# catniplab/vlgp

Hardware: AMD Instinct MI355X
Metric: EM iterations/sec (higher is better)
Workload: dtype f64

## Files before the change

### vlgp_amd/csrc/api.hip

```cpp
#include <stdarg.h>
#include <stdio.h>
#include <stdlib.h>
#include <string.h>

#include <chrono>

#include <algorithm>
#include <new>

#include "ctx.h"

static thread_local std::string g_create_err;

int vlgp_fail(vlgp_ctx* ctx, int code, const char* fmt, ...) {
    char buf[1024];
    va_list ap;
    va_start(ap, fmt);
    vsnprintf(buf, sizeof(buf), fmt, ap);
    va_end(ap);
    if (ctx) ctx->err = buf;
    else g_create_err = buf;
    return code;
}

// ... 117 lines not shown
    if (us->is(a.kinds)) return VLGP_OK;
    if (us->is(SET_REPLICATED) && &a != &admit_vlgp_replicate)
        return vlgp_fail(ctx, VLGP_ERR_STATE, "%s refuses a replicated set (leave-one-out replicas of set %d: "
                         "E-step, download, loglik and free only)", a.what, us->rep.src);
    return vlgp_fail(ctx, VLGP_ERR_STATE, a.refusal, set);
}

enum : unsigned {
    OPEN_COLLECT = 1,
    OPEN_STALE = 2,
    OPEN_JOIN = 4,
    OPEN_WAIT = 8,
    OPEN_PARAMS = 16,
    OPEN_DEVICE = 32,
    OPEN_EMPTY = 64,
};
#define NEED_PARAMS(ctx) \
    if (!(ctx)->have_params) return vlgp_fail(ctx, VLGP_ERR_STATE, "parameters not set (vlgp_set_params)")
static int open_set(vlgp_ctx* ctx, int set, unsigned how, UnitSet** out, const Admission* a) {
    NEED_CTX(ctx);
    if (how & OPEN_COLLECT) CHK(vlgp_prior_collect(ctx));
    if (how & OPEN_STALE) ctx->hmom_us = nullptr;
    if (how & OPEN_JOIN) CHK(vlgp_join_m(ctx));
    if (how & OPEN_WAIT) {
        CHK(wait_norms(ctx));
        if (ctx->m_pending) HIPCHK(ctx, hipEventSynchronize(ctx->ev_m_done));
    }
    if (how & OPEN_PARAMS) NEED_PARAMS(ctx);
    if (how & OPEN_DEVICE) HIPCHK(ctx, hipSetDevice(ctx->dev));
    if (!(*out = vlgp_get_set(ctx, set, !(how & OPEN_EMPTY)))) return VLGP_ERR_ARG;
    return a ? admit(ctx, set, *out, *a) : VLGP_OK;
}
static int open_pair(vlgp_ctx* ctx, int src, int dst, bool bad_args, const char* bad, UnitSet** s, UnitSet** d) {
    CHK(open_set(ctx, src, OPEN_STALE | OPEN_JOIN | OPEN_DEVICE, s, nullptr));
    if (!(*d = vlgp_get_set(ctx, dst, false))) return VLGP_ERR_ARG;
// ... 51 lines not shown

static void free_set(vlgp_ctx* ctx, UnitSet& us) {
    if (!us.valid) return;
    (void)hipStreamSynchronize(ctx->stream);
    auto fr = [](void* p) { if (p) (void)hipFree(p); };
    if (us.is(SET_REPLICATED)) {
        Replicas& r = us.rep;
        fr(us.mu); fr(us.v); fr(us.w); fr(r.d_ch); fr(r.d_pair); fr(r.d_mask); fr(r.d_wconst); fr(r.d_nobs); fr(r.d_xa);
        ctx->sets[r.src].rep_users--;
        us.d_xb = nullptr;
    } else if (!us.alias) {
        fr(us.y); fr(us.x); fr(us.mu); fr(us.v); fr(us.w);
    }
    fr(us.dmu); fr(us.d_off); fr(us.d_src_start); fr(us.d_unit_prior); fr(us.d_xb); fr(us.d_scratch); fr(us.d_mu_stash);
    fr(us.d_links);
    us = UnitSet();
}

static void free_with_tiling_cuts(vlgp_ctx* ctx, int set) {
    for (auto& other : ctx->sets)
        if (other.valid && other.is(SET_TILING) && other.parent == set) free_set(ctx, other);
    free_set(ctx, ctx->sets[set]);
}

extern "C" int vlgp_create(int device, int N, int L, int P, int R, const uint8_t* gauss_mask, vlgp_ctx** out) {
    if (!out) return vlgp_fail(nullptr, VLGP_ERR_ARG, "null output handle");
    *out = nullptr;
    if (N < 1 || L < 1 || P < 1 || R < 1) return vlgp_fail(nullptr, VLGP_ERR_ARG, "N, L, P, R must be positive");
    if (R > VLGP_MAX_RANK) return vlgp_fail(nullptr, VLGP_ERR_ARG, "rank %d exceeds VLGP_MAX_RANK=%d", R, VLGP_MAX_RANK);
    if (L > VLGP_MAX_L) return vlgp_fail(nullptr, VLGP_ERR_ARG, "at most %d latents supported, got %d", VLGP_MAX_L, L);
// ... 740 lines not shown
            return vlgp_fail(ctx, VLGP_ERR_STATE, "no prior factor for unit length %d (call build_prior/set_prior)", T);
        idx[m] = it->second.index;
    }
    HIPCHK(ctx, hipMemcpy(us.d_unit_prior, idx.data(), sizeof(int) * us.M, hipMemcpyHostToDevice));
    us.prior_epoch = ctx->prior_epoch;
    return VLGP_OK;
}

int vlgp_refresh_xb(vlgp_ctx* ctx, UnitSet& us) {
    if (us.x_ones) return VLGP_OK;
    if (!us.d_xb) HIPCHK(ctx, hipMalloc(&us.d_xb, (size_t)us.rows * ctx->N * sizeof(double)));
    return launch_xb(ctx, us);
}

static int begin_count(vlgp_ctx* ctx) {
    HIPCHK(ctx, hipMemsetAsync(ctx->d_fail, 0, sizeof(int), ctx->stream));
    return VLGP_OK;
}
static int end_count(vlgp_ctx* ctx, int* n_failed) {
    if (!n_failed) return VLGP_OK;
    HIPCHK(ctx, hipMemcpyAsync(n_failed, ctx->d_fail, sizeof(int), hipMemcpyDeviceToHost, ctx->stream));
    HIPCHK(ctx, hipStreamSynchronize(ctx->stream));
    return VLGP_OK;
}

extern "C" int vlgp_update_w(vlgp_ctx* ctx, int set) {
    UnitSet* us = nullptr;
    CHK(open_set(ctx, set, OPEN_COLLECT | OPEN_STALE | OPEN_JOIN | OPEN_PARAMS | OPEN_DEVICE, &us, &admit_vlgp_update_w));
    return launch_estep(ctx, *us, EM_W, 0, 0.0, 0);
}

extern "C" int vlgp_update_v(vlgp_ctx* ctx, int set, int vb, int* n_failed) {
    UnitSet* us = nullptr;
    CHK(open_set(ctx, set, OPEN_COLLECT | OPEN_JOIN | OPEN_PARAMS | OPEN_DEVICE, &us, &admit_vlgp_update_v));
    if (n_failed) *n_failed = 0;
    if (!vb) return VLGP_OK;
    CHK(begin_count(ctx));
    CHK(launch_estep(ctx, *us, EM_FACTOR0 | EM_V, 0, 0.0, 1));
    return end_count(ctx, n_failed);
}

static int estep_staged(vlgp_ctx* ctx, UnitSet& us, int mode, int n_iter, double dmu_bound, int vb) {
    const int W = us.Tmax, N = ctx->N, L = ctx->L, P = ctx->P;
    CHK(vlgp_bind_priors(ctx, us));
    const int n_stages = (int)us.stage_start.size() - 1;
    for (int s = 0; s < n_stages; ++s) {
        const int u0 = us.stage_start[s], cnt = us.stage_start[s + 1] - u0;
        if (cnt < 1) continue;
        CHK(launch_links_copy(ctx, us, us.link_start[s], us.link_start[s + 1], 0));
        UnitSet v;
        v.valid = true; v.M = cnt; v.rows = (int64_t)cnt * W; v.Tmax = v.Tmin = W;
        v.off.resize(cnt + 1);
        for (int m = 0; m <= cnt; ++m) v.off[m] = (int64_t)m * W;
        v.d_off = us.d_off;
        const int64_t r0 = (int64_t)u0 * W;
        v.y = us.y + r0 * N; v.x = us.x ? us.x + r0 * P * N : nullptr;
        v.mu = us.mu + r0 * L; v.v = us.v + r0 * L; v.w = us.w + r0 * L; v.dmu = us.dmu + r0 * L;
        v.x_ones = us.x_ones; v.alias = true;
// ... 1 lines not shown
        if (!us.x_ones) {
            if (!us.d_xb) HIPCHK(ctx, hipMalloc(&us.d_xb, (size_t)us.rows * N * sizeof(double)));
            v.d_xb = us.d_xb + r0 * N;
        }
        v.d_scratch = us.d_scratch; v.scratch_len = us.scratch_len;
        const int rc = launch_estep(ctx, v, mode, n_iter, dmu_bound, vb);
        us.d_scratch = v.d_scratch; us.scratch_len = v.scratch_len;
        if (rc != VLGP_OK) return rc;
        CHK(launch_links_copy(ctx, us, us.link_start[s], us.link_start[s + 1], 1));
    }
    return VLGP_OK;
}

extern "C" int vlgp_estep(vlgp_ctx* ctx, int set, int n_iter, double dmu_bound, int vb, int* n_failed) {
    UnitSet* us = nullptr;
    CHK(open_set(ctx, set, OPEN_COLLECT | OPEN_STALE | OPEN_JOIN | OPEN_PARAMS | OPEN_DEVICE, &us, &admit_vlgp_estep));
    if (n_failed) *n_failed = 0;
    if (n_iter < 1) return VLGP_OK;
    if (!(dmu_bound > 0)) return vlgp_fail(ctx, VLGP_ERR_ARG, "dmu_bound must be positive");
    CHK(begin_count(ctx));
    const int mode = EM_FACTOR0 | EM_MEAN | EM_W | (vb ? EM_V : 0);
    if (us->stage_start.size() > 2) CHK(estep_staged(ctx, *us, mode, n_iter, dmu_bound, vb ? 1 : 0));
    else CHK(launch_estep(ctx, *us, mode, n_iter, dmu_bound, vb ? 1 : 0));
    if (!ctx->ev_e_done) HIPCHK(ctx, hipEventCreateWithFlags(&ctx->ev_e_done, hipEventDisableTiming));
    HIPCHK(ctx, hipEventRecord(ctx->ev_e_done, ctx->stream));
    ctx->e_done_valid = true;
    return end_count(ctx, n_failed);
}

extern "C" int vlgp_set_overlaps(vlgp_ctx* ctx, int set, int n_stages, const int* stage_start, int n_links,
                                 const int* links, const int* link_start) {
// ... 142 lines not shown
        ctx->last_h_ms = std::chrono::duration<double, std::milli>(std::chrono::steady_clock::now().time_since_epoch()).count() - ctx->h_t0;
    ctx->hmom_bracket = false;
    ctx->hmom_us = nullptr;
    ctx->hwlm_valid = false;
    return VLGP_OK;
}

extern "C" int vlgp_apply_latent_map(vlgp_ctx* ctx, int set, const double* map, const double* shift) {
    NEED_CTX(ctx);
    ctx->hmom_us = nullptr;
    CHK(vlgp_join_m(ctx));
    HIPCHK(ctx, hipSetDevice(ctx->dev));
    UnitSet* us = vlgp_get_set(ctx, set, true);
    if (!us || !map) return vlgp_fail(ctx, VLGP_ERR_ARG, "bad latent map arguments");
    CHK(admit(ctx, set, us, admit_vlgp_apply_latent_map));
    const int L = ctx->L;
    if (!ctx->h_stage_map) {
        HIPCHK(ctx, hipHostMalloc(&ctx->h_stage_map, sizeof(double) * (L * L + L + 8), hipHostMallocDefault));
        HIPCHK(ctx, hipMalloc(&ctx->d_stage_map, sizeof(double) * (L * L + L + 8)));
        HIPCHK(ctx, hipEventCreateWithFlags(&ctx->ev_stage_map, hipEventDisableTiming));
    }
    if (ctx->stage_map_busy) HIPCHK(ctx, hipEventSynchronize(ctx->ev_stage_map));
    memcpy(ctx->h_stage_map, map, sizeof(double) * L * L);
    if (shift) memcpy(ctx->h_stage_map + L * L, shift, sizeof(double) * L);
    HIPCHK(ctx, hipMemcpyAsync(ctx->d_stage_map, ctx->h_stage_map, sizeof(double) * (L * L + L), hipMemcpyHostToDevice, ctx->stream));
    const double* d_map = ctx->d_stage_map;
    const double* d_shift = shift ? ctx->d_stage_map + L * L : nullptr;
    CHK(launch_latent_map(ctx, *us, d_map, d_shift));
    CHK(launch_links_map(ctx, *us, d_map, d_shift));
    HIPCHK(ctx, hipEventRecord(ctx->ev_stage_map, ctx->stream));
    ctx->stage_map_busy = true;
    return VLGP_OK;
}

static int moments_host(vlgp_ctx* ctx, UnitSet& us, std::vector<double>& out) {
    const int L = ctx->L;
    const int K = L * (L + 1) / 2 + 3 * L + 1;
    CHK(vlgp_ensure_pinned(ctx, K + 8));
    CHK(launch_moments(ctx, us));
    HIPCHK(ctx, hipMemcpyAsync(ctx->h_pinned, ctx->d_work, sizeof(double) * K, hipMemcpyDeviceToHost, ctx->stream));
    HIPCHK(ctx, hipStreamSynchronize(ctx->stream));
    out.assign(ctx->h_pinned, ctx->h_pinned + K);
// ... 274 lines not shown
```

### vlgp_amd/csrc/ctx.h

```cpp
#pragma once
#include <hip/hip_runtime.h>
#include <stdint.h>

#include <map>
#include <string>
#include <vector>

#include "../../include/vlgp_hip.h"

#define VLGP_WAVE 64
#define VLGP_E_LANES 4
#define VLGP_PRIOR_SLOTS 64

struct Prior {
    int T = 0;
    double* d_full = nullptr;
    double* d_compact = nullptr;
    std::vector<int> rl;
    std::vector<int64_t> goff;
    int64_t compact_len = 0;
    int index = -1;
};

enum : unsigned {
// ... 157 lines not shown
    double* d_hres = nullptr;
    unsigned h_seq = 0;
    double* d_hmpart = nullptr;
    bool hprep = false;
    hipEvent_t ev_e_done = nullptr;
    bool e_done_valid = false;
    uint64_t hprep_epoch = 0, write_epoch = 0;
    double* d_hmom = nullptr;
    int64_t hmom_len = 0;
    const UnitSet* hmom_us = nullptr;
    int hmom_T = 0;
    bool hmom_bracket = false;
    double* d_hwlm = nullptr;
    int64_t hwlm_len = 0;
    bool hwlm_valid = false;
    struct LrThr { int T; double dt, tol; std::vector<double> om; };
    std::vector<LrThr> lr_thr;
    Switches sw;
    std::vector<const void*> lds_attr_done;
    int h_prio = 1;
    double last_h_ms = 0.0, last_m_ms = 0.0;
    double h_t0 = 0.0;
    int last_hstep_path = 0;
    double hstat[4] = {0.0, 0.0, 0.0, 0.0};

    bool prof_on = false;
    ProfSlot prof[VLGP_PROF_KINDS];
    hipEvent_t ev0 = nullptr, ev1 = nullptr;
    struct PendingProf { int kind; hipEvent_t a, b; double units; bool done; };
    std::vector<PendingProf> pending;
// ... 9 lines not shown

    double* d_xwork = nullptr;
    double* h_xres = nullptr;
    double* d_xres = nullptr;
    unsigned long long x_seq = 0;
    int x_pending = 0;
    int x_set = -1;
    double* h_msnap = nullptr;
    double* d_msnap = nullptr;
    bool msnap_valid = false;
    double* h_stage_par = nullptr;
    double* h_stage_map = nullptr;
    double* d_stage_map = nullptr;
    hipEvent_t ev_stage_par = nullptr, ev_stage_map = nullptr;
    bool stage_par_busy = false, stage_map_busy = false;

    double* d_elbo = nullptr;
    int64_t elbo_len = 0;

    std::string err;
};

inline UnitSet& vlgp_rows_owner(vlgp_ctx* ctx, UnitSet& us) { return us.rep.src >= 0 ? ctx->sets[us.rep.src] : us; }

struct LoglikShape { int64_t slots, n_rate; int grid_y; const char* limit; };
inline LoglikShape vlgp_loglik_shape(const vlgp_ctx* ctx, const UnitSet& us) {
    if (us.is(SET_BY_ROW))
        return {(int64_t)us.rep.n * ctx->N, us.rep.rows_src * ctx->N, us.rep.n, "vlgp_loglik: at most 65535 replicas per masked set"};
    if (us.is(SET_GROUPS))
        return {us.rep.n_pairs, us.rep.rows_src * us.rep.n_pairs, us.rep.n_pairs,
// ... 48 lines not shown
static_assert(EP_LEN == VLGP_ESTEP_PLAN_LEN, "vlgp_debug_estep_plan: the report's length is part of the ABI");
int launch_mstep(vlgp_ctx* ctx, UnitSet& us, int n_iter, int use_hessian, double eps, double lr,
                 double da_bound, double db_bound);
int mstep_plan_report(vlgp_ctx* ctx, int64_t rows, int out[12]);
int launch_hstep(vlgp_ctx* ctx, UnitSet& us, int window, double dt, int n_eval, const int* latent,
                 const double* logp, double* ll, double* dll);
int launch_ichol_all(vlgp_ctx* ctx, const std::vector<Prior*>& prs, const double* omega, const double* sigma,
                     bool in_table, bool lazy = false);
int vlgp_prior_collect(vlgp_ctx* ctx);
int launch_compact_prior(vlgp_ctx* ctx, Prior& pr);
int launch_sample_posterior(vlgp_ctx* ctx, int T, int n, const double* d_mu, const double* d_w, const double* d_G,
                            const double* d_eps, double* d_z, double* d_out);
int launch_npx_probe(vlgp_ctx* ctx, int kind, int64_t n, const double* d_a, const double* d_b, double* d_out);
int launch_xb(vlgp_ctx* ctx, UnitSet& us);
int launch_latent_map(vlgp_ctx* ctx, UnitSet& us, const double* d_map, const double* d_shift);
int launch_snapshot_params(vlgp_ctx* ctx, hipStream_t st, double* d_host);
int launch_norms(vlgp_ctx* ctx, UnitSet& us, double* d_part, unsigned* d_ticket, double* d_host, unsigned long long seq);
int launch_links_copy(vlgp_ctx* ctx, UnitSet& us, int l0, int l1, int dir);
int launch_links_map(vlgp_ctx* ctx, UnitSet& us, const double* d_map, const double* d_shift);
int hstep_prepare(vlgp_ctx* ctx, UnitSet& us, int T, hipStream_t st);
int launch_moments(vlgp_ctx* ctx, UnitSet& us);
int launch_project(vlgp_ctx* ctx, UnitSet& us, const double* d_proj, const double* d_shift, double* d_part,
                   double* d_out);
int launch_gather(vlgp_ctx* ctx, UnitSet& src, UnitSet& dst, int window);
int launch_loglik(vlgp_ctx* ctx, UnitSet& us, int vb, double* d_rate, double* d_sums);
int launch_sums_finish(vlgp_ctx* ctx, int slots, int n_blk, const double* d_part, double* d_sums);
int launch_scatter(vlgp_ctx* ctx, UnitSet& cut, UnitSet& dst, int window);
int launch_elbo(vlgp_ctx* ctx, UnitSet& us, int vb, int rp, double* d_part, double* d_sums, double* d_row_ell,
                double* d_terms, int* d_flag);
int launch_forecast(vlgp_ctx* ctx, UnitSet& us, int vb, int rp, double* d_z, const int64_t* d_ext_off,
// ... 3 lines not shown
```

### vlgp_amd/csrc/estep.hip

```cpp
#include "ctx.h"

#include "estep_args.h"
#include "fast_exp.h"

__device__ __forceinline__ void wave_sync() {
    __builtin_amdgcn_fence(__ATOMIC_ACQ_REL, "workgroup");
    __builtin_amdgcn_wave_barrier();
}

__device__ __forceinline__ double shfl_xor_f64(double x, int m) { return __shfl_xor(x, m, 64); }

enum { PASS_YA = 0, PASS_RES = 1, PASS_W = 2 };

template <bool SMALL, int LT>
__global__ void __launch_bounds__(SMALL ? 512 : 1024) estep_kernel(EstepArgs A) {
    extern __shared__ __attribute__((aligned(16))) double smem[];
    const int tid = threadIdx.x, nthr = blockDim.x;
    const int lane = tid & 63, wid = tid >> 6, nw = nthr >> 6;
    const int N = A.N, L = A.L;
    const int m = blockIdx.x;
    const int64_t r0 = A.off[m];
    const int T = (int)(A.off[m + 1] - r0);
    const int pidx = A.unit_prior ? A.unit_prior[m] : -1;
    const double* Gbase = pidx >= 0 ? A.prior_base[pidx] : nullptr;
// ... 370 lines not shown

struct SmallPlan { bool fits; int nthr; int64_t d; };
static SmallPlan plan_generic_small(const UnitSet& us, int L, int64_t common, int64_t gsz, int64_t lcsz, int64_t ints,
                                    int64_t lds_max) {
    const int nw_s = L < 4 ? 4 : (L > 8 ? 8 : L);
    const int64_t small_d = common + 2LL * nw_s * 64 + 6LL * us.Tmax * L + gsz + lcsz + ints;
    return SmallPlan{us.Tmax <= 256 && small_d * 8 <= lds_max, nw_s * 64, small_d};
}

int launch_estep(vlgp_ctx* ctx, UnitSet& us, int mode, int n_iter, double dmu_bound, int vb, int* report) {
    const int N = ctx->N, L = ctx->L;
    const bool need_prior = (mode & (EM_FACTOR0 | EM_MEAN | EM_V)) != 0;
    if (need_prior) CHK(vlgp_bind_priors(ctx, us));
    if (report) {
    } else {
        UnitSet& src = vlgp_rows_owner(ctx, us);
        if (!src.x_ones) CHK(vlgp_refresh_xb(ctx, src));
        us.d_xb = src.d_xb;
    }

    const RankSummary rs = need_prior ? estep_rank_summary(ctx, us) : RankSummary();
    const int64_t gsz = rs.g_odd, lcsz = rs.lc_odd;

    const int64_t LDS_MAX = 160 * 1024;
    const int LTl = generic_lt(L);
    const int64_t common = 2LL * LTl * N + 2LL * N + ((L + 1) & ~1);
    const int64_t ints = ((int64_t)N + 4 * L + 1) / 2 + 1;

    EstepArgs A;
    A.N = N; A.L = L;
// ... 5 lines not shown
    A.a = ctx->d_a; A.b = ctx->d_b; A.noise = ctx->d_noise; A.gauss = ctx->d_gauss;
    A.scratch = nullptr; A.lc_global = nullptr; A.lc_stride = 0;
    A.fail = ctx->d_fail;
    A.clk = ctx->d_clk;
    A.cols_g = nullptr; A.wconst_g = nullptr;
    A.lds_T = us.Tmax; A.lds_gsz = (int)gsz; A.lds_lcsz = (int)lcsz;

    int* path = report ? &report[EP_FAMILY] : &ctx->last_estep_path;

    {
        int handled = 0;
        CHK(launch_estep_split(ctx, us, A, rs, &handled, report));
        if (handled) { *path = handled == 2 ? VLGP_PATH_ESTEP_LSPLIT : (handled == 3 ? VLGP_PATH_ESTEP_SPLIT_MIXED : VLGP_PATH_ESTEP_SPLIT); return VLGP_OK; }
        if (us.is(SET_REPLICATED))
            return vlgp_fail(ctx, VLGP_ERR_STATE, "replicated set: only the split E-step leaves a channel out, and it declined");
    }

    {
        int handled = 0;
        CHK(launch_estep_fast(ctx, us, A, rs, &handled, report));
        if (handled) { *path = VLGP_PATH_ESTEP_FAST; return VLGP_OK; }
    }

    if (us.Tmax > 64) {
        int handled = 0;
        CHK(launch_estep_long(ctx, us, A, &handled, report));
        if (handled) { *path = VLGP_PATH_ESTEP_LONG; return VLGP_OK; }
    }

    const SmallPlan sp = plan_generic_small(us, L, common, gsz, lcsz, ints, LDS_MAX);
// ... 51 lines not shown
```

### vlgp_amd/csrc/estep_split.hip

```cpp
#include <stdlib.h>
#include <string.h>

#include <algorithm>

#include <type_traits>

#include "estep_args.h"
#include "wave_tri.h"
#include "fast_exp.h"

namespace {

enum { SP_YA = 0, SP_RES = 1, SP_W = 2 };
typedef double double4_t __attribute__((ext_vector_type(4)));

struct ExclArgs;
struct SplitArgs {
    int N, L, M;
    int64_t rows;
    const int64_t* off;
    const int* unit_prior;
    const double* const* prior_base;
    const int* prior_rl;
    const int64_t* prior_goff;
// ... 32 lines not shown
struct ExclArgs {
    const unsigned long long* mask;
    const double* wconst;
    const double* y;
    const double* xb;
    int64_t rows_src;
    int64_t row_base;
    const double* mu_lm;
};
__host__ __device__ inline int excl_words(int N) { return (N + 63) >> 6; }
enum { EX_BY_ROW = 64 };

template <int LT>
constexpr int rec_len() { return (2 * LT + 3 + 1) & ~1; }

__global__ void __launch_bounds__(256)
esplit_cols_kernel(int N, int L, int LT, int REC, const double* __restrict__ a, const double* __restrict__ b,
                   const double* __restrict__ noise, const int* __restrict__ gauss, double* __restrict__ cols,
                   double* __restrict__ wconst, double* __restrict__ ycoef) {
    __shared__ int order[1024];
    __shared__ int gs[1024];
    __shared__ double cinv[1024];
    for (int n = threadIdx.x; n < N; n += 256) {
        const int g = gauss[n];
        gs[n] = g;
        cinv[n] = g ? 1.0 / noise[n] : 1.0;
    }
    __syncthreads();
    {
        int total = 0;
        for (int m = 0; m < N; ++m) total += gs[m];
        for (int n = threadIdx.x; n < N; n += 256) {
            int c = 0;
            for (int m = 0; m < n; ++m) c += gs[m];
// ... 55 lines not shown
__global__ void __launch_bounds__(256)
esplit_row_wconst(int N, int L, int64_t rows, int nw, const double* __restrict__ a, const double* __restrict__ noise,
                  const int* __restrict__ gauss, const unsigned long long* __restrict__ mask,
                  double* __restrict__ wconst) {
    const int64_t row = (int64_t)blockIdx.x * 256 + threadIdx.x;
    if (row >= rows) return;
    const unsigned long long* mk = mask + row * nw;
    for (int l = 0; l < L; ++l) {
        double s = 0.0;
        for (int n = 0; n < N; ++n)
            if (gauss[n] && !((mk[n >> 6] >> (n & 63)) & 1ull)) s = fma(a[l * N + n] * a[l * N + n], 1.0 / noise[n], s);
        wconst[row * L + l] = s;
    }
}

__global__ void __launch_bounds__(256)
esplit_to_lm(int L, int64_t rows, const double* __restrict__ a0, const double* __restrict__ a1,
             const double* __restrict__ a2, double* __restrict__ b0, double* __restrict__ b1, double* __restrict__ b2) {
    const int64_t row = (int64_t)blockIdx.x * 256 + threadIdx.x;
    if (row >= rows) return;
    for (int l = 0; l < L; ++l) {
        const double x0 = a0[row * L + l], x1 = a1[row * L + l], x2 = a2[row * L + l];
        b0[l * rows + row] = x0;
        b1[l * rows + row] = x1;
        b2[l * rows + row] = x2;
    }
}
__global__ void __launch_bounds__(256)
esplit_from_lm(int L, int64_t rows, const double* __restrict__ b0, const double* __restrict__ b1,
               const double* __restrict__ b2, double* a0, double* a1, double* a2) {
    const int64_t i = (int64_t)blockIdx.x * 256 + threadIdx.x;
    if (i >= rows * L) return;
    const int64_t row = i / L, l = i - row * L;
    const int64_t src = l * rows + row;
    a0[i] = b0[src];
    a1[i] = b1[src];
    a2[i] = b2[src];
}
// ... 1701 lines not shown
    const int N = ctx->N, L = ctx->L, LT = P.LT, pkg = P.pkg, n_lanes = P.n_lanes, n_it = P.n_it;
    const bool lng = P.lng;
    const LatentClasses& C = P.C;
    const int64_t nRL = P.nRL;
    if (us.scratch_len < P.scratch_len) {
        if (us.d_scratch) HIPCHK(ctx, hipFree(us.d_scratch));
        us.d_scratch = nullptr;
        us.scratch_len = 0;
        HIPCHK(ctx, hipMalloc(&us.d_scratch, (size_t)P.scratch_len * 8));
        us.scratch_len = P.scratch_len;
    }
    if (!ctx->d_ecols) HIPCHK(ctx, hipMalloc(&ctx->d_ecols, sizeof(double) * ((size_t)N * 50 + 32)));
    double* cols = ctx->d_ecols;
    double* wconst = ctx->d_ecols + (int64_t)N * 34;
    double* ycoef = wconst + 32;
    hipLaunchKernelGGL(esplit_cols_kernel, dim3(1), dim3(256), 0, ctx->stream, N, L, LT, P.REC, ctx->d_a, ctx->d_b,
                       ctx->d_noise, ctx->d_gauss, cols, wconst, ycoef);
    HIPCHK(ctx, hipGetLastError());
    ExclArgs XA{};
    if (rep) {
        XA.mask = us.rep.d_mask;
        XA.wconst = us.rep.d_wconst;
        XA.y = vlgp_rows_owner(ctx, us).y;
        XA.xb = E.xb;
        XA.rows_src = us.rep.rows_src;
        XA.row_base = 0;
        XA.mu_lm = nullptr;
        if (!by_row)
            hipLaunchKernelGGL(esplit_excl_wconst, dim3((unsigned)((us.rep.n * 16 + 255) / 256)), dim3(256), 0, ctx->stream, N,
                               L, us.rep.n, us.rep.nw, ctx->d_a, ctx->d_noise, ctx->d_gauss, us.rep.d_mask, us.rep.d_wconst);
        else if (us.rep.d_wconst)
            hipLaunchKernelGGL(esplit_row_wconst, dim3((unsigned)((us.rows + 255) / 256)), dim3(256), 0, ctx->stream, N, L,
                               us.rows, us.rep.nw, ctx->d_a, ctx->d_noise, ctx->d_gauss, us.rep.d_mask, us.rep.d_wconst);
        HIPCHK(ctx, hipGetLastError());
    }

    SplitArgs A;
    A.N = N; A.L = L; A.M = us.M; A.rows = us.rows;
    A.off = E.off; A.unit_prior = E.unit_prior; A.prior_base = E.prior_base; A.prior_rl = E.prior_rl;
    A.prior_goff = E.prior_goff;
    A.y = E.y; A.xb = E.xb; A.dmu = E.dmu;
    A.ld = us.rows;
    A.ra = us.d_scratch; A.ya = A.ra + nRL; A.mu = A.ya + nRL; A.v = A.mu + nRL; A.w = A.v + nRL;
    A.xg = A.w + nRL; A.pkg = pkg;
    {
        const unsigned nb = (unsigned)((us.rows + 255) / 256);
        hipLaunchKernelGGL(esplit_to_lm, dim3(nb), dim3(256), 0, ctx->stream, L, us.rows, E.mu, E.v, E.w, A.mu, A.v, A.w);
        HIPCHK(ctx, hipGetLastError());
    }
    if (rep) {
        XA.mu_lm = A.mu;
        static_assert(sizeof(ExclArgs) <= sizeof(us.rep.xh), "Replicas::xh too small for ExclArgs");
        memcpy(us.rep.xh, &XA, sizeof(ExclArgs));
        HIPCHK(ctx, hipMemcpyAsync(us.rep.d_xa, us.rep.xh, sizeof(ExclArgs), hipMemcpyHostToDevice, ctx->stream));
    }
    A.failg = reinterpret_cast<int*>(us.d_scratch + P.o_failg);
    A.xl = us.d_scratch + P.o_xl;
    A.sv = P.use_lane ? A.xl + P.xl_len : nullptr;
    A.dl = P.use_lane ? A.sv + nRL : nullptr;
    A.dmask = 0;
    A.fail = E.fail;
    A.wconst = wconst;
    A.dmu_bound = E.dmu_bound;
    A.ntot = N; A.np = N - ctx->n_gauss;
    A.lds_g = 256; A.pkl = pkg; A.n_lat = 0;
    A.shg = 0; A.shg_cap = 0; A.shg_T = 0;
    A.do_v = 0; A.last = 0;
    *handled = split_handled(P);
    HIPCHK(ctx, hipMemsetAsync(A.failg, 0, sizeof(int) * (size_t)us.M * L, ctx->stream));

    const int mode = E.mode;
    const bool with_mean = (mode & EM_MEAN) != 0;
    const int kind = lng ? VLGP_PROF_ESTEP_LONG
                         : (P.maxra <= 16 ? VLGP_PROF_ESTEP_RA16 : (P.maxra <= 24 ? VLGP_PROF_ESTEP_RA24 : VLGP_PROF_ESTEP_RA32));
    vlgp_prof_begin(ctx, kind);
    Lane main_lane{ctx->stream, rep ? &XA : nullptr, rep ? reinterpret_cast<const ExclArgs*>(us.rep.d_xa) : nullptr, by_row};
    int rc = VLGP_OK;
    if (with_mean) rc = run_ya(ctx, main_lane, A, LT, cols, ycoef);

    for (int h = 1; h < n_lanes; ++h) {
        if (ctx->elane[h - 1]) continue;
        HIPCHK(ctx, hipStreamCreateWithFlags(&ctx->elane[h - 1], hipStreamNonBlocking));
        HIPCHK(ctx, hipEventCreateWithFlags(&ctx->ev_e_join[h - 1], hipEventDisableTiming));
    }
// ... 64 lines not shown
                hf.lat.do_v = do_v ? 1 : 0;
                if (sample) vlgp_prof_begin(ctx, VLGP_PROF_ESTEP_FACTOR, ln.st);
                rc = lng ? run_latent_long(ctx, ln, hf.lat, false) : run_latent(ctx, ln, hf.lat, C, false);
                if (sample) vlgp_prof_end(ctx, VLGP_PROF_ESTEP_FACTOR, tasks, ln.st);
            }
        }
    }
    for (int h = 1; h < n_lanes; ++h) {
        (void)hipEventRecord(ctx->ev_e_join[h - 1], ctx->elane[h - 1]);
        (void)hipStreamWaitEvent(ctx->stream, ctx->ev_e_join[h - 1], 0);
    }
    if (rc == VLGP_OK) {
        const unsigned nb = (unsigned)((nRL + 255) / 256);
        hipLaunchKernelGGL(esplit_from_lm, dim3(nb), dim3(256), 0, ctx->stream, L, us.rows, A.mu, A.v, A.w, E.mu, E.v, E.w);
        if (hipGetLastError() != hipSuccess) rc = vlgp_fail(ctx, VLGP_ERR_HIP, "esplit_from_lm launch failed");
    }
    vlgp_prof_end(ctx, kind, (double)us.M * (E.n_iter > 0 ? E.n_iter : 1));
    return rc;
}
```

### vlgp_amd/csrc/hstep.hip

```cpp
#include <stdio.h>
#include <stdlib.h>
#include <string.h>

#include <algorithm>

#include "ctx.h"
#include "wave_tri.h"
#include "hstep_mfma.h"
#include "hstep_lr.h"

#define HS_MAXT 1024

struct HPrepArgs {
    int T;
    double dt;
    const double* logp;
    double* kinv;
    double* q;
    double* dk;
    double* scal;
    double* tm;
    double* km;
};

// ... 500 lines not shown
    const int64_t* off;
    const double* mu;
    const double* w;
    const double* wlm;
    int64_t wld;
    int latent[16];
    double logp[48];
    double* kinv;
    double* kcol;
    double* scal;
    double* out;
};

template <int T>
__global__ void __launch_bounds__(256) hstep_moment_kernel(int L, int M, int Tr, const int64_t* off, const double* mu,
                                                           int nchunk, double* part) {
    constexpr int CW = (T * T + 255) / 256;
    constexpr int NG = (T + CW - 1) / CW;
    static_assert(T * NG <= 256, "one thread per (row, run)");
    constexpr int SG = 16;
    __shared__ __attribute__((aligned(16))) double s[SG][64];
    const int l = blockIdx.y, c = blockIdx.x, tid = threadIdx.x;
    const int per = (M + nchunk - 1) / nchunk;
    const int m0 = c * per, m1 = (m0 + per < M) ? m0 + per : M;
    const bool act = tid < T * NG;
    const int j = act ? tid % T : 0, k0 = act ? (tid / T) * CW : 0;
    double acc[CW];
#pragma unroll
    for (int i = 0; i < CW; ++i) acc[i] = 0.0;
    const int w4 = tid >> 6, t = tid & 63;
    double nx[SG / 4];
    auto fetch = [&](int m) {
#pragma unroll
        for (int q = 0; q < SG / 4; ++q) {
            const int sg = w4 + 4 * q;
            nx[q] = (m + sg < m1 && t < Tr) ? mu[(off[m + sg] + t) * L + l] : 0.0;
        }
    };
    if (m0 < m1) fetch(m0);
    for (int m = m0; m < m1; m += SG) {
        __syncthreads();
#pragma unroll
        for (int q = 0; q < SG / 4; ++q) s[w4 + 4 * q][t] = nx[q];
        __syncthreads();
        if (m + SG < m1) fetch(m + SG);
#pragma unroll
        for (int sg = 0; sg < SG; ++sg) {
            const double a = s[sg][j];
#pragma unroll
            for (int i = 0; i < CW; ++i) acc[i] = fma(a, (k0 + i < 64) ? s[sg][k0 + i] : 0.0, acc[i]);
        }
// ... 389 lines not shown
    return VLGP_OK;
}

static int launch_hstep_impl(vlgp_ctx* ctx, UnitSet& us, int window, double dt, int n_eval, const int* latent,
                             const double* logp, double* ll, double* dll, bool force_dense);

int launch_hstep(vlgp_ctx* ctx, UnitSet& us, int window, double dt, int n_eval, const int* latent,
                 const double* logp, double* ll, double* dll) {
    return launch_hstep_impl(ctx, us, window, dt, n_eval, latent, logp, ll, dll, false);
}

static bool hstep_round_kernels_apply(vlgp_ctx* ctx, const UnitSet& us, int T) {
    const Switches& sw = ctx->sw;
    return us.Tmin == T && us.Tmax == T && T <= 64 && T >= (sw.hstep_dense ? 24 : 4) && !sw.hstep_generic;
}
static int hstep_prepare_units(vlgp_ctx* ctx, UnitSet& us, int T, bool want_wlm, bool want_mom, hipStream_t st) {
    const int L = ctx->L, M = us.M;
    if (want_wlm && (!ctx->hwlm_valid || ctx->hmom_us != &us)) {
        const int64_t n = us.rows * L;
        if (ctx->hwlm_len < n) {
            if (ctx->d_hwlm) HIPCHK(ctx, hipFree(ctx->d_hwlm));
            ctx->d_hwlm = nullptr; ctx->hwlm_len = 0;
            HIPCHK(ctx, hipMalloc(&ctx->d_hwlm, sizeof(double) * (size_t)n));
            ctx->hwlm_len = n;
        }
        hipLaunchKernelGGL(hstep_w_latent_major, dim3((unsigned)((n + 255) / 256)), dim3(256), 0, st, L,
                           us.rows, us.w, ctx->d_hwlm);
        HIPCHK(ctx, hipGetLastError());
        ctx->hwlm_valid = true;
    }
    if (!want_mom) return VLGP_OK;
    const int HT = T <= 50 ? 50 : 64;
    constexpr int NCH = 64;
    if (!ctx->d_hmom || ctx->hmom_len < (int64_t)L * HT * HT) {
        if (ctx->d_hmom) HIPCHK(ctx, hipFree(ctx->d_hmom));
        if (ctx->d_hmpart) HIPCHK(ctx, hipFree(ctx->d_hmpart));
        ctx->d_hmom = nullptr; ctx->d_hmpart = nullptr;
        HIPCHK(ctx, hipMalloc(&ctx->d_hmom, sizeof(double) * L * HT * HT));
        HIPCHK(ctx, hipMalloc(&ctx->d_hmpart, sizeof(double) * (size_t)L * NCH * HT * HT));
        ctx->hmom_len = (int64_t)L * HT * HT;
        ctx->hmom_us = nullptr;
    }
    if (ctx->hmom_us != &us || ctx->hmom_T != T) {
        if (HT == 50)
            hipLaunchKernelGGL((hstep_moment_kernel<50>), dim3(NCH, L), dim3(256), 0, st, L, M, T,
                               us.d_off, us.mu, NCH, ctx->d_hmpart);
        else
            hipLaunchKernelGGL((hstep_moment_kernel<64>), dim3(NCH, L), dim3(256), 0, st, L, M, T,
                               us.d_off, us.mu, NCH, ctx->d_hmpart);
        hipLaunchKernelGGL(hstep_moment_reduce, dim3((HT * HT + 255) / 256, L), dim3(256), 0, st, NCH,
                           HT * HT, ctx->d_hmpart, ctx->d_hmom);
        HIPCHK(ctx, hipGetLastError());
        ctx->hmom_us = &us;
        ctx->hmom_T = T;
    }
    return VLGP_OK;
}
int hstep_prepare(vlgp_ctx* ctx, UnitSet& us, int T, hipStream_t st) {
    if (!hstep_round_kernels_apply(ctx, us, T)) return VLGP_OK;
    ctx->hmom_us = nullptr;
    ctx->hwlm_valid = false;
    return hstep_prepare_units(ctx, us, T, !ctx->sw.hstep_no_wlm, true, st);
}

static int launch_hstep_impl(vlgp_ctx* ctx, UnitSet& us, int window, double dt, int n_eval, const int* latent,
                             const double* logp, double* ll, double* dll, bool force_dense) {
    const int T = window, L = ctx->L, M = us.M;
    if (T > HS_MAXT) return vlgp_fail(ctx, VLGP_ERR_ARG, "H-step kernel supports window <= %d, got %d", HS_MAXT, T);
    const bool huge = (size_t)(T * (T | 1)) * 8 > 150 * 1024;
    if (us.Tmin != T || us.Tmax != T)
        return vlgp_fail(ctx, VLGP_ERR_STATE, "H-step needs every unit to have exactly window=%d rows", T);
    const Switches& sw = ctx->sw;
    const bool lr_allowed = !force_dense && !sw.hstep_dense;
    const bool fast = T <= 64 && T >= (lr_allowed ? 4 : 24) && !sw.hstep_generic;
    const int TC = T <= 50 ? 50 : 64;
    const int64_t TT = fast ? (int64_t)TC * TC : (int64_t)T * T;
    const int64_t o_kinv = 0, o_q = o_kinv + n_eval * TT, o_dk = o_q + n_eval * TT, o_scal = o_dk + n_eval * TT;
// ... 11 lines not shown
    double* W = ctx->d_work;
    double* hp = ctx->h_pinned;
    if (n_eval > 16) return vlgp_fail(ctx, VLGP_ERR_ARG, "at most 16 evaluations per call, got %d", n_eval);
    for (int i = 0; i < n_eval; ++i)
        if (latent[i] < 0 || latent[i] >= L) return vlgp_fail(ctx, VLGP_ERR_ARG, "latent index out of range");

    if (fast) {
        HFastArgs F;
        F.L = L; F.M = M; F.Tr = T; F.dt = dt; F.off = us.d_off; F.mu = us.mu; F.w = us.w;
        for (int i = 0; i < n_eval; ++i) F.latent[i] = latent[i];
        for (int i = 0; i < 3 * n_eval; ++i) F.logp[i] = logp[i];
        F.kinv = W + o_kinv; F.kcol = W + o_q; F.scal = W + o_scal; F.out = W + o_out;
        F.wlm = nullptr; F.wld = 0;
        if (ctx->hmom_bracket && !sw.hstep_no_wlm) {
            CHK(hstep_prepare_units(ctx, us, T, true, false, ctx->stream));
            F.wlm = ctx->d_hwlm; F.wld = us.rows;
        }
        double* hres = hp + 4 * n_eval + 8;
        {
            if (!ctx->d_hsync) {
                HIPCHK(ctx, hipMalloc(&ctx->d_hsync, 32 * sizeof(unsigned)));
                HIPCHK(ctx, hipMemsetAsync(ctx->d_hsync, 0, 32 * sizeof(unsigned), ctx->stream));
                HIPCHK(ctx, hipHostMalloc(&ctx->h_hres, 64 * sizeof(double), hipHostMallocMapped));
                memset(ctx->h_hres, 0, 64 * sizeof(double));
                HIPCHK(ctx, hipHostGetDevicePointer(reinterpret_cast<void**>(&ctx->d_hres), ctx->h_hres, 0));
            }
            if (!ctx->hmom_bracket) ctx->hmom_us = nullptr;
            CHK(hstep_prepare_units(ctx, us, T, false, true, ctx->stream));
            HRoundArgs R;
            R.F = F;
            constexpr int MFMA_NW = 4;
// ... 274 lines not shown
```

### vlgp_amd/engine.py

```python
import collections
import ctypes as C
import logging
import os
import time

import numpy as np

from . import _lib
from ._lib import VlgpError, check, dptr, i64ptr, iptr, u8ptr

logger = logging.getLogger(__name__)

__all__ = ["Engine", "DeviceTrials", "estep", "mstep", "hstep", "update_w", "update_v",
           "make_cholesky", "infer", "vem", "constrain_loading", "constrain_latent", "VlgpError"]


TRACE = {}


def _f64(a):
    return np.ascontiguousarray(a, dtype=np.float64)


def _all_ones(x):
# ... 842 lines not shown
    def begin_m():
        if params.get("da") is None:
            params["da"] = np.zeros_like(params["a"])
            params["db"] = np.zeros_like(params["b"])
        eng.mstep_begin(sid, config["Mniter"], config["use_hessian"], config["eps"], config["learning_rate"],
                        config["da_bound"], config["db_bound"])

    early_m = m_async and not latent_constraint and not track_elbo
    if early_m:
        begin_m()
    m_first = m_async and ((eng.world > 1 and not eng.host_exchange) or bool(os.environ.get("VLGP_M_SEQUENTIAL")))

    prepare = bool(config["Hstep"]) and bool(config.get("window")) and not m_first

    def after_estep():
        eng.norms_begin(sid)
        if prepare:
            eng.hstep_prepare(sid, config["window"])

    if not latent_constraint:
        after_estep()
    eng.estep_wait()
    t1 = time.perf_counter()
    elbo_now = _elbo_totals(eng, sid, config["method"] == "VB") if track_elbo else None
    constrain_latent(trials, params, config)
    if latent_constraint:
        after_estep()
    norms_epoch = eng.state_epoch
    if m_async and not early_m:
        begin_m()

    def finish_m():
        bad, ms = eng.mstep_end()
# ... 55 lines not shown
```

Before: 154.6.

## Defer latent map and fuse it with fail-clear into split E-step prologue

The latent-map application is deferred and folded into a new fused prologue kernel that combines the column setup, the transpose to latent-major layout and the clearing of the failure counters. This removes several small launches and memsets per EM iteration. The H-step preparation now reuses the latent-major mu and w copies left behind by the split E-step instead of re-transposing them, and hstep_prepare is reordered before norms_begin. The deferral bookkeeping adds state that must be flushed correctly on every other entry path.

```diff
diff --git a/vlgp_amd/csrc/api.hip b/vlgp_amd/csrc/api.hip
--- a/vlgp_amd/csrc/api.hip
+++ b/vlgp_amd/csrc/api.hip
@@ -155,11 +155,28 @@
     OPEN_PARAMS = 16,
     OPEN_DEVICE = 32,
     OPEN_EMPTY = 64,
+    OPEN_KEEP_MAP = 128,
 };
+
+int vlgp_flush_latent_map(vlgp_ctx* ctx) {
+    if (ctx->map_pending < 0) return VLGP_OK;
+    UnitSet& us = ctx->sets[ctx->map_pending];
+    HIPCHK(ctx, hipSetDevice(ctx->dev));
+    const int L = ctx->L;
+    CHK(launch_latent_map(ctx, us, ctx->d_stage_map, ctx->map_shift ? ctx->d_stage_map + L * L : nullptr));
+    return vlgp_latent_map_consumed(ctx);
+}
+int vlgp_latent_map_consumed(vlgp_ctx* ctx) {
+    ctx->map_pending = -1;
+    HIPCHK(ctx, hipEventRecord(ctx->ev_stage_map, ctx->stream));
+    ctx->stage_map_busy = true;
+    return VLGP_OK;
+}
 #define NEED_PARAMS(ctx) \
     if (!(ctx)->have_params) return vlgp_fail(ctx, VLGP_ERR_STATE, "parameters not set (vlgp_set_params)")
 static int open_set(vlgp_ctx* ctx, int set, unsigned how, UnitSet** out, const Admission* a) {
     NEED_CTX(ctx);
+    if (!(how & OPEN_KEEP_MAP)) CHK(vlgp_flush_latent_map(ctx));
     if (how & OPEN_COLLECT) CHK(vlgp_prior_collect(ctx));
     if (how & OPEN_STALE) ctx->hmom_us = nullptr;
     if (how & OPEN_JOIN) CHK(vlgp_join_m(ctx));
@@ -241,6 +258,8 @@
     }
     fr(us.dmu); fr(us.d_off); fr(us.d_src_start); fr(us.d_unit_prior); fr(us.d_xb); fr(us.d_scratch); fr(us.d_mu_stash);
     fr(us.d_links);
+    if (ctx->lm.us == &us) ctx->lm.us = nullptr;
+    if (ctx->hwlm != ctx->d_hwlm) ctx->hwlm_valid = false;
     us = UnitSet();
 }
 
@@ -1011,10 +1030,14 @@
 }
 
 static int begin_count(vlgp_ctx* ctx) {
-    HIPCHK(ctx, hipMemsetAsync(ctx->d_fail, 0, sizeof(int), ctx->stream));
+    ctx->fail_clear = true;
     return VLGP_OK;
 }
 static int end_count(vlgp_ctx* ctx, int* n_failed) {
+    if (ctx->fail_clear) {
+        ctx->fail_clear = false;
+        HIPCHK(ctx, hipMemsetAsync(ctx->d_fail, 0, sizeof(int), ctx->stream));
+    }
     if (!n_failed) return VLGP_OK;
     HIPCHK(ctx, hipMemcpyAsync(n_failed, ctx->d_fail, sizeof(int), hipMemcpyDeviceToHost, ctx->stream));
     HIPCHK(ctx, hipStreamSynchronize(ctx->stream));
@@ -1023,13 +1046,13 @@
 
 extern "C" int vlgp_update_w(vlgp_ctx* ctx, int set) {
     UnitSet* us = nullptr;
-    CHK(open_set(ctx, set, OPEN_COLLECT | OPEN_STALE | OPEN_JOIN | OPEN_PARAMS | OPEN_DEVICE, &us, &admit_vlgp_update_w));
+    CHK(open_set(ctx, set, OPEN_COLLECT | OPEN_STALE | OPEN_JOIN | OPEN_PARAMS | OPEN_DEVICE | OPEN_KEEP_MAP, &us, &admit_vlgp_update_w));
     return launch_estep(ctx, *us, EM_W, 0, 0.0, 0);
 }
 
 extern "C" int vlgp_update_v(vlgp_ctx* ctx, int set, int vb, int* n_failed) {
     UnitSet* us = nullptr;
-    CHK(open_set(ctx, set, OPEN_COLLECT | OPEN_JOIN | OPEN_PARAMS | OPEN_DEVICE, &us, &admit_vlgp_update_v));
+    CHK(open_set(ctx, set, OPEN_COLLECT | OPEN_JOIN | OPEN_PARAMS | OPEN_DEVICE | OPEN_KEEP_MAP, &us, &admit_vlgp_update_v));
     if (n_failed) *n_failed = 0;
     if (!vb) return VLGP_OK;
     CHK(begin_count(ctx));
@@ -1039,6 +1062,7 @@
 
 static int estep_staged(vlgp_ctx* ctx, UnitSet& us, int mode, int n_iter, double dmu_bound, int vb) {
     const int W = us.Tmax, N = ctx->N, L = ctx->L, P = ctx->P;
+    CHK(vlgp_flush_latent_map(ctx));
     CHK(vlgp_bind_priors(ctx, us));
     const int n_stages = (int)us.stage_start.size() - 1;
     for (int s = 0; s < n_stages; ++s) {
@@ -1070,7 +1094,7 @@
 
 extern "C" int vlgp_estep(vlgp_ctx* ctx, int set, int n_iter, double dmu_bound, int vb, int* n_failed) {
     UnitSet* us = nullptr;
-    CHK(open_set(ctx, set, OPEN_COLLECT | OPEN_STALE | OPEN_JOIN | OPEN_PARAMS | OPEN_DEVICE, &us, &admit_vlgp_estep));
+    CHK(open_set(ctx, set, OPEN_COLLECT | OPEN_STALE | OPEN_JOIN | OPEN_PARAMS | OPEN_DEVICE | OPEN_KEEP_MAP, &us, &admit_vlgp_estep));
     if (n_failed) *n_failed = 0;
     if (n_iter < 1) return VLGP_OK;
     if (!(dmu_bound > 0)) return vlgp_fail(ctx, VLGP_ERR_ARG, "dmu_bound must be positive");
@@ -1243,6 +1267,7 @@
     UnitSet* us = vlgp_get_set(ctx, set, true);
     if (!us || !map) return vlgp_fail(ctx, VLGP_ERR_ARG, "bad latent map arguments");
     CHK(admit(ctx, set, us, admit_vlgp_apply_latent_map));
+    CHK(vlgp_flush_latent_map(ctx));
     const int L = ctx->L;
     if (!ctx->h_stage_map) {
         HIPCHK(ctx, hipHostMalloc(&ctx->h_stage_map, sizeof(double) * (L * L + L + 8), hipHostMallocDefault));
@@ -1255,6 +1280,11 @@
     HIPCHK(ctx, hipMemcpyAsync(ctx->d_stage_map, ctx->h_stage_map, sizeof(double) * (L * L + L), hipMemcpyHostToDevice, ctx->stream));
     const double* d_map = ctx->d_stage_map;
     const double* d_shift = shift ? ctx->d_stage_map + L * L : nullptr;
+    if (us->n_links == 0 && us->stage_start.size() <= 2) {
+        ctx->map_pending = set;
+        ctx->map_shift = shift != nullptr;
+        return VLGP_OK;
+    }
     CHK(launch_latent_map(ctx, *us, d_map, d_shift));
     CHK(launch_links_map(ctx, *us, d_map, d_shift));
     HIPCHK(ctx, hipEventRecord(ctx->ev_stage_map, ctx->stream));
diff --git a/vlgp_amd/csrc/ctx.h b/vlgp_amd/csrc/ctx.h
--- a/vlgp_amd/csrc/ctx.h
+++ b/vlgp_amd/csrc/ctx.h
@@ -195,6 +195,10 @@
     double* d_hwlm = nullptr;
     int64_t hwlm_len = 0;
     bool hwlm_valid = false;
+    const double* hwlm = nullptr;
+    struct LmCopy { const UnitSet* us; uint64_t epoch; const double *mu, *w; int64_t ld; };
+    LmCopy lm = {nullptr, 0, nullptr, nullptr, 0};
+    bool fail_clear = false;
     struct LrThr { int T; double dt, tol; std::vector<double> om; };
     std::vector<LrThr> lr_thr;
     Switches sw;
@@ -234,6 +238,8 @@
     double* d_stage_map = nullptr;
     hipEvent_t ev_stage_par = nullptr, ev_stage_map = nullptr;
     bool stage_par_busy = false, stage_map_busy = false;
+    int map_pending = -1;
+    bool map_shift = false;
 
     double* d_elbo = nullptr;
     int64_t elbo_len = 0;
@@ -312,6 +318,8 @@
 int launch_npx_probe(vlgp_ctx* ctx, int kind, int64_t n, const double* d_a, const double* d_b, double* d_out);
 int launch_xb(vlgp_ctx* ctx, UnitSet& us);
 int launch_latent_map(vlgp_ctx* ctx, UnitSet& us, const double* d_map, const double* d_shift);
+int vlgp_flush_latent_map(vlgp_ctx* ctx);
+int vlgp_latent_map_consumed(vlgp_ctx* ctx);
 int launch_snapshot_params(vlgp_ctx* ctx, hipStream_t st, double* d_host);
 int launch_norms(vlgp_ctx* ctx, UnitSet& us, double* d_part, unsigned* d_ticket, double* d_host, unsigned long long seq);
 int launch_links_copy(vlgp_ctx* ctx, UnitSet& us, int l0, int l1, int dir);
diff --git a/vlgp_amd/csrc/estep.hip b/vlgp_amd/csrc/estep.hip
--- a/vlgp_amd/csrc/estep.hip
+++ b/vlgp_amd/csrc/estep.hip
@@ -408,6 +408,9 @@
     if (need_prior) CHK(vlgp_bind_priors(ctx, us));
     if (report) {
     } else {
+        if (ctx->hwlm_valid && ctx->hwlm != ctx->d_hwlm) ctx->hwlm_valid = false;
+        ctx->lm.us = nullptr;
+        if (ctx->map_pending >= 0 && &ctx->sets[ctx->map_pending] != &us) CHK(vlgp_flush_latent_map(ctx));
         UnitSet& src = vlgp_rows_owner(ctx, us);
         if (!src.x_ones) CHK(vlgp_refresh_xb(ctx, src));
         us.d_xb = src.d_xb;
@@ -443,6 +446,11 @@
         if (handled) { *path = handled == 2 ? VLGP_PATH_ESTEP_LSPLIT : (handled == 3 ? VLGP_PATH_ESTEP_SPLIT_MIXED : VLGP_PATH_ESTEP_SPLIT); return VLGP_OK; }
         if (us.is(SET_REPLICATED))
             return vlgp_fail(ctx, VLGP_ERR_STATE, "replicated set: only the split E-step leaves a channel out, and it declined");
+        if (!report) CHK(vlgp_flush_latent_map(ctx));
+        if (!report && ctx->fail_clear) {
+            ctx->fail_clear = false;
+            HIPCHK(ctx, hipMemsetAsync(ctx->d_fail, 0, sizeof(int), ctx->stream));
+        }
     }
 
     {
diff --git a/vlgp_amd/csrc/estep_split.hip b/vlgp_amd/csrc/estep_split.hip
--- a/vlgp_amd/csrc/estep_split.hip
+++ b/vlgp_amd/csrc/estep_split.hip
@@ -70,10 +70,10 @@
 template <int LT>
 constexpr int rec_len() { return (2 * LT + 3 + 1) & ~1; }
 
-__global__ void __launch_bounds__(256)
-esplit_cols_kernel(int N, int L, int LT, int REC, const double* __restrict__ a, const double* __restrict__ b,
-                   const double* __restrict__ noise, const int* __restrict__ gauss, double* __restrict__ cols,
-                   double* __restrict__ wconst, double* __restrict__ ycoef) {
+__device__ __forceinline__ void
+esplit_cols_block(int N, int L, int LT, int REC, const double* __restrict__ a, const double* __restrict__ b,
+                  const double* __restrict__ noise, const int* __restrict__ gauss, double* __restrict__ cols,
+                  double* __restrict__ wconst, double* __restrict__ ycoef) {
     __shared__ int order[1024];
     __shared__ int gs[1024];
     __shared__ double cinv[1024];
@@ -159,14 +159,48 @@
     }
 }
 
+template <int LT>
 __global__ void __launch_bounds__(256)
-esplit_to_lm(int L, int64_t rows, const double* __restrict__ a0, const double* __restrict__ a1,
-             const double* __restrict__ a2, double* __restrict__ b0, double* __restrict__ b1, double* __restrict__ b2) {
-    const int64_t row = (int64_t)blockIdx.x * 256 + threadIdx.x;
+esplit_prologue(int N, int L, int REC, const double* __restrict__ a, const double* __restrict__ b,
+                const double* __restrict__ noise, const int* __restrict__ gauss, double* __restrict__ cols,
+                double* __restrict__ wconst, double* __restrict__ ycoef, int64_t rows, double* a0,
+                const double* __restrict__ a1, const double* __restrict__ a2, double* __restrict__ b0,
+                double* __restrict__ b1, double* __restrict__ b2, int* __restrict__ failg, int64_t n_failg,
+                int* __restrict__ fail, const double* __restrict__ map, const double* __restrict__ shift) {
+    if (blockIdx.x == 0) {
+        esplit_cols_block(N, L, LT, REC, a, b, noise, gauss, cols, wconst, ycoef);
+        return;
+    }
+    __shared__ double m_s[LT * LT], s_s[LT];
+    if (map) {
+        for (int i = threadIdx.x; i < L * L; i += 256) m_s[i] = map[i];
+        for (int i = threadIdx.x; i < L; i += 256) s_s[i] = shift ? shift[i] : 0.0;
+        __syncthreads();
+    }
+    const int64_t t0 = (int64_t)(blockIdx.x - 1) * 256 + threadIdx.x, nt = (int64_t)(gridDim.x - 1) * 256;
+    if (t0 == 0 && fail) *fail = 0;
+    for (int64_t i = t0; i < n_failg; i += nt) failg[i] = 0;
+    const int64_t row = t0;
     if (row >= rows) return;
+    if (map) {
+        double in[LT];
+#pragma unroll
+        for (int l = 0; l < LT; ++l) in[l] = l < L ? a0[row * L + l] - s_s[l] : 0.0;
+#pragma unroll
+        for (int c = 0; c < LT; ++c) {
+            if (c < L) {
+                double s = 0.0;
+#pragma unroll
+                for (int l = 0; l < LT; ++l)
+                    if (l < L) s = fma(in[l], m_s[l * L + c], s);
+                a0[row * L + c] = s;
+                b0[c * rows + row] = s;
+            }
+        }
+    }
     for (int l = 0; l < L; ++l) {
-        const double x0 = a0[row * L + l], x1 = a1[row * L + l], x2 = a2[row * L + l];
-        b0[l * rows + row] = x0;
+        const double x1 = a1[row * L + l], x2 = a2[row * L + l];
+        if (!map) b0[l * rows + row] = a0[row * L + l];
         b1[l * rows + row] = x1;
         b2[l * rows + row] = x2;
     }
@@ -1898,9 +1932,30 @@
     double* cols = ctx->d_ecols;
     double* wconst = ctx->d_ecols + (int64_t)N * 34;
     double* ycoef = wconst + 32;
-    hipLaunchKernelGGL(esplit_cols_kernel, dim3(1), dim3(256), 0, ctx->stream, N, L, LT, P.REC, ctx->d_a, ctx->d_b,
-                       ctx->d_noise, ctx->d_gauss, cols, wconst, ycoef);
-    HIPCHK(ctx, hipGetLastError());
+    SplitArgs A;
+    A.ld = us.rows;
+    A.ra = us.d_scratch; A.ya = A.ra + nRL; A.mu = A.ya + nRL; A.v = A.mu + nRL; A.w = A.v + nRL;
+    A.failg = reinterpret_cast<int*>(us.d_scratch + P.o_failg);
+    {
+        const unsigned nb = (unsigned)((us.rows + 255) / 256);
+        int* fail_clear = ctx->fail_clear ? ctx->d_fail : nullptr;
+        ctx->fail_clear = false;
+        const bool fold = ctx->map_pending >= 0;
+        const double* d_map = fold ? ctx->d_stage_map : nullptr;
+        const double* d_shift = fold && ctx->map_shift ? ctx->d_stage_map + L * L : nullptr;
+        const dim3 grid((nb < 1 ? 1 : nb) + 1), blk(256);
+#define PROLOGUE(LTV)                                                                                                      \
+        hipLaunchKernelGGL((esplit_prologue<LTV>), grid, blk, 0, ctx->stream, N, L, P.REC, ctx->d_a, ctx->d_b, ctx->d_noise, \
+                           ctx->d_gauss, cols, wconst, ycoef, us.rows, E.mu, E.v, E.w, A.mu, A.v, A.w, A.failg,             \
+                           (int64_t)us.M * L, fail_clear, d_map, d_shift)
+        if (LT == 3) PROLOGUE(3);
+        else if (LT == 5) PROLOGUE(5);
+        else if (LT == 8) PROLOGUE(8);
+        else PROLOGUE(10);
+#undef PROLOGUE
+        HIPCHK(ctx, hipGetLastError());
+        if (fold) CHK(vlgp_latent_map_consumed(ctx));
+    }
     ExclArgs XA{};
     if (rep) {
         XA.mask = us.rep.d_mask;
@@ -1919,26 +1974,17 @@
         HIPCHK(ctx, hipGetLastError());
     }
 
-    SplitArgs A;
     A.N = N; A.L = L; A.M = us.M; A.rows = us.rows;
     A.off = E.off; A.unit_prior = E.unit_prior; A.prior_base = E.prior_base; A.prior_rl = E.prior_rl;
     A.prior_goff = E.prior_goff;
     A.y = E.y; A.xb = E.xb; A.dmu = E.dmu;
-    A.ld = us.rows;
-    A.ra = us.d_scratch; A.ya = A.ra + nRL; A.mu = A.ya + nRL; A.v = A.mu + nRL; A.w = A.v + nRL;
     A.xg = A.w + nRL; A.pkg = pkg;
-    {
-        const unsigned nb = (unsigned)((us.rows + 255) / 256);
-        hipLaunchKernelGGL(esplit_to_lm, dim3(nb), dim3(256), 0, ctx->stream, L, us.rows, E.mu, E.v, E.w, A.mu, A.v, A.w);
-        HIPCHK(ctx, hipGetLastError());
-    }
     if (rep) {
         XA.mu_lm = A.mu;
         static_assert(sizeof(ExclArgs) <= sizeof(us.rep.xh), "Replicas::xh too small for ExclArgs");
         memcpy(us.rep.xh, &XA, sizeof(ExclArgs));
         HIPCHK(ctx, hipMemcpyAsync(us.rep.d_xa, us.rep.xh, sizeof(ExclArgs), hipMemcpyHostToDevice, ctx->stream));
     }
-    A.failg = reinterpret_cast<int*>(us.d_scratch + P.o_failg);
     A.xl = us.d_scratch + P.o_xl;
     A.sv = P.use_lane ? A.xl + P.xl_len : nullptr;
     A.dl = P.use_lane ? A.sv + nRL : nullptr;
@@ -1951,7 +1997,6 @@
     A.shg = 0; A.shg_cap = 0; A.shg_T = 0;
     A.do_v = 0; A.last = 0;
     *handled = split_handled(P);
-    HIPCHK(ctx, hipMemsetAsync(A.failg, 0, sizeof(int) * (size_t)us.M * L, ctx->stream));
 
     const int mode = E.mode;
     const bool with_mean = (mode & EM_MEAN) != 0;
@@ -2046,6 +2091,8 @@
         const unsigned nb = (unsigned)((nRL + 255) / 256);
         hipLaunchKernelGGL(esplit_from_lm, dim3(nb), dim3(256), 0, ctx->stream, L, us.rows, A.mu, A.v, A.w, E.mu, E.v, E.w);
         if (hipGetLastError() != hipSuccess) rc = vlgp_fail(ctx, VLGP_ERR_HIP, "esplit_from_lm launch failed");
+        else if ((uintptr_t)&us >= (uintptr_t)ctx->sets && (uintptr_t)&us < (uintptr_t)(ctx->sets + VLGP_MAX_SETS))
+            ctx->lm = {&us, ctx->write_epoch, A.mu, A.w, A.ld};
     }
     vlgp_prof_end(ctx, kind, (double)us.M * (E.n_iter > 0 ? E.n_iter : 1));
     return rc;
diff --git a/vlgp_amd/csrc/hstep.hip b/vlgp_amd/csrc/hstep.hip
--- a/vlgp_amd/csrc/hstep.hip
+++ b/vlgp_amd/csrc/hstep.hip
@@ -538,7 +538,7 @@
 
 template <int T>
 __global__ void __launch_bounds__(256) hstep_moment_kernel(int L, int M, int Tr, const int64_t* off, const double* mu,
-                                                           int nchunk, double* part) {
+                                                           int64_t mrs, int64_t mls, int nchunk, double* part) {
     constexpr int CW = (T * T + 255) / 256;
     constexpr int NG = (T + CW - 1) / CW;
     static_assert(T * NG <= 256, "one thread per (row, run)");
@@ -558,7 +558,7 @@
 #pragma unroll
         for (int q = 0; q < SG / 4; ++q) {
             const int sg = w4 + 4 * q;
-            nx[q] = (m + sg < m1 && t < Tr) ? mu[(off[m + sg] + t) * L + l] : 0.0;
+            nx[q] = (m + sg < m1 && t < Tr) ? mu[(off[m + sg] + t) * mrs + l * mls] : 0.0;
         }
     };
     if (m0 < m1) fetch(m0);
@@ -978,9 +978,14 @@
     const Switches& sw = ctx->sw;
     return us.Tmin == T && us.Tmax == T && T <= 64 && T >= (sw.hstep_dense ? 24 : 4) && !sw.hstep_generic;
 }
-static int hstep_prepare_units(vlgp_ctx* ctx, UnitSet& us, int T, bool want_wlm, bool want_mom, hipStream_t st) {
+static int hstep_prepare_units(vlgp_ctx* ctx, UnitSet& us, int T, bool want_wlm, bool want_mom, hipStream_t st,
+                               bool from_lm = false) {
     const int L = ctx->L, M = us.M;
-    if (want_wlm && (!ctx->hwlm_valid || ctx->hmom_us != &us)) {
+    const bool lm = from_lm && ctx->lm.us == &us && ctx->lm.epoch == ctx->write_epoch && ctx->lm.ld == us.rows;
+    if (want_wlm && (!ctx->hwlm_valid || ctx->hmom_us != &us) && lm) {
+        ctx->hwlm = ctx->lm.w;
+        ctx->hwlm_valid = true;
+    } else if (want_wlm && (!ctx->hwlm_valid || ctx->hmom_us != &us)) {
         const int64_t n = us.rows * L;
         if (ctx->hwlm_len < n) {
             if (ctx->d_hwlm) HIPCHK(ctx, hipFree(ctx->d_hwlm));
@@ -991,6 +996,7 @@
         hipLaunchKernelGGL(hstep_w_latent_major, dim3((unsigned)((n + 255) / 256)), dim3(256), 0, st, L,
                            us.rows, us.w, ctx->d_hwlm);
         HIPCHK(ctx, hipGetLastError());
+        ctx->hwlm = ctx->d_hwlm;
         ctx->hwlm_valid = true;
     }
     if (!want_mom) return VLGP_OK;
@@ -1006,12 +1012,14 @@
         ctx->hmom_us = nullptr;
     }
     if (ctx->hmom_us != &us || ctx->hmom_T != T) {
+        const double* mu = lm ? ctx->lm.mu : us.mu;
+        const int64_t mrs = lm ? 1 : L, mls = lm ? ctx->lm.ld : 1;
         if (HT == 50)
             hipLaunchKernelGGL((hstep_moment_kernel<50>), dim3(NCH, L), dim3(256), 0, st, L, M, T,
-                               us.d_off, us.mu, NCH, ctx->d_hmpart);
+                               us.d_off, mu, mrs, mls, NCH, ctx->d_hmpart);
         else
             hipLaunchKernelGGL((hstep_moment_kernel<64>), dim3(NCH, L), dim3(256), 0, st, L, M, T,
-                               us.d_off, us.mu, NCH, ctx->d_hmpart);
+                               us.d_off, mu, mrs, mls, NCH, ctx->d_hmpart);
         hipLaunchKernelGGL(hstep_moment_reduce, dim3((HT * HT + 255) / 256, L), dim3(256), 0, st, NCH,
                            HT * HT, ctx->d_hmpart, ctx->d_hmom);
         HIPCHK(ctx, hipGetLastError());
@@ -1024,7 +1032,7 @@
     if (!hstep_round_kernels_apply(ctx, us, T)) return VLGP_OK;
     ctx->hmom_us = nullptr;
     ctx->hwlm_valid = false;
-    return hstep_prepare_units(ctx, us, T, !ctx->sw.hstep_no_wlm, true, st);
+    return hstep_prepare_units(ctx, us, T, !ctx->sw.hstep_no_wlm, true, st, true);
 }
 
 static int launch_hstep_impl(vlgp_ctx* ctx, UnitSet& us, int window, double dt, int n_eval, const int* latent,
@@ -1066,7 +1074,7 @@
         F.wlm = nullptr; F.wld = 0;
         if (ctx->hmom_bracket && !sw.hstep_no_wlm) {
             CHK(hstep_prepare_units(ctx, us, T, true, false, ctx->stream));
-            F.wlm = ctx->d_hwlm; F.wld = us.rows;
+            F.wlm = ctx->hwlm; F.wld = us.rows;
         }
         double* hres = hp + 4 * n_eval + 8;
         {
diff --git a/vlgp_amd/engine.py b/vlgp_amd/engine.py
--- a/vlgp_amd/engine.py
+++ b/vlgp_amd/engine.py
@@ -880,9 +880,9 @@
     prepare = bool(config["Hstep"]) and bool(config.get("window")) and not m_first
 
     def after_estep():
-        eng.norms_begin(sid)
         if prepare:
             eng.hstep_prepare(sid, config["window"])
+        eng.norms_begin(sid)
 
     if not latent_constraint:
         after_estep()
```

After: 154.7, median of 4. About the same (+0.1%).
